# intel/hexl-fpga

Measured on AMD Instinct MI355X. Metric: keyswitches/sec at N=16384, decomp=7, higher is better.
Workload: dtype u64; 1 GPU; keyswitch N=16384 decomp_modulus_size=7 key_modulus_size=8 52-bit primes (GeneratePrimes(K,51,N)), kcc=2, batch 8192 per step split over 1 GPU(s) (8192 on rank 0), resident in HBM; global_batch=8192, batch_per_gpu=8192, parallelism=1 independent shard(s), no collective

## Files before the change

### hexl-fpga_amd/__init__.py

```python
from __future__ import annotations

import ctypes
import os
import subprocess
from pathlib import Path

import numpy as np

_PKG = Path(__file__).resolve().parent
ROOT = _PKG.parent
LIB_PATH = Path(os.environ["HEXL_MI355X_LIB"]) if os.environ.get("HEXL_MI355X_LIB") else _PKG / "lib" / "libhexl_mi355x.so"

_u64 = ctypes.c_uint64
_sz = ctypes.c_size_t
_vp = ctypes.c_void_p
_i = ctypes.c_int

C_ABI = {
    "hexl_device_count": [],
    "hexl_ctx_create": [_i, ctypes.POINTER(_vp)],
    "hexl_ctx_destroy": [_vp],
    "hexl_ctx_set_stream": [_vp, _vp],
    "hexl_ctx_use_own_stream": [_vp],
    "hexl_ctx_sync": [_vp],
    "hexl_ctx_describe": [_vp, ctypes.c_char_p, _sz],
    "hexl_ntt_fwd": [_vp, _vp, _sz, _vp, _vp, _u64, _u64],
    "hexl_ntt_inv": [_vp, _vp, _sz, _vp, _vp, _u64, _u64, _u64, _u64],
    "hexl_dyadic_multiply": [_vp, _vp, _vp, _vp, _sz, _u64, _vp, _u64],
    "hexl_ks_plan_create": [_vp, _u64, _u64, _u64, _u64, _u64, _vp, _vp, _vp, ctypes.POINTER(_vp)],
    "hexl_ks_plan_destroy": [_vp],
    "hexl_ks_set_keys": [_vp, ctypes.POINTER(_vp)],
    "hexl_keyswitch": [_vp, _vp, _vp, _sz],
    "hexl_ks_range_check": [_vp],
    "hexl_ks_plan_tiers": [_vp, ctypes.POINTER(_i)],
    "hexl_multiply_relinearize": [_vp, _vp, _vp, _vp, _sz],
    "hexl_apply_galois": [_vp, _vp, _vp, _sz, _u64, _u64],
    "hexl_rescale": [_vp, _vp, _vp, _sz, _u64, _u64],
    "hexl_rotate": [_vp, _vp, _vp, _sz, _u64],
    "hexl_rotate_hoisted": [ctypes.POINTER(_vp), ctypes.POINTER(_u64), _sz, ctypes.POINTER(_vp), _vp, _sz],
    "hexl_linear_transform": [ctypes.POINTER(_vp), ctypes.POINTER(_u64), ctypes.POINTER(_vp), _sz, _vp, _vp, _vp, _sz],
    "hexl_linear_transform_bsgs": [ctypes.POINTER(_vp), ctypes.POINTER(_u64), _sz, ctypes.POINTER(_vp), ctypes.POINTER(_u64), _sz,
                                   ctypes.POINTER(_vp), ctypes.POINTER(_vp), _vp, _vp, _sz],
    "hexl_lt_bsgs_scratch_bytes": [_vp, _sz, _sz],
    "hexl_rns_ntt_fwd": [_vp, _vp, _vp, _sz, _u64],
    "hexl_rns_ntt_inv": [_vp, _vp, _vp, _sz, _u64],
    "hexl_multiply_plain": [_vp, _vp, _vp, _vp, _sz, _u64, _u64, _sz, _i],
    "hexl_ks_scratch_bytes": [_vp, _sz],
    "hexl_ntt_fwd_host": [_vp, ctypes.POINTER(_vp), _sz, _vp, _vp, _u64, _u64],
    "hexl_ntt_inv_host": [_vp, ctypes.POINTER(_vp), _sz, _vp, _vp, _u64, _u64, _u64, _u64],
    "hexl_dyadic_multiply_host": [_vp, ctypes.POINTER(_vp), ctypes.POINTER(_vp), ctypes.POINTER(_vp), _sz, _u64,
                                  ctypes.POINTER(_vp), _u64],
    "hexl_keyswitch_host": [_vp, ctypes.POINTER(_vp), ctypes.POINTER(_vp), _sz],
    "hexl_ks_time_stages": [_vp, _vp, _vp, _sz, _i, ctypes.POINTER(ctypes.c_float)],
}


class HexlError(RuntimeError):
    pass


def build(force: bool = False) -> Path:
    if force or not LIB_PATH.exists():
        subprocess.run(["make", "-C", str(_PKG / "csrc"), "-j4"] + (["-B"] if force else []), check=True)
    else:
        subprocess.run(["make", "-C", str(_PKG / "csrc"), "-j4", "-s"], check=True)
    return LIB_PATH

# ... 96 lines not shown
    def __init__(self, ctx: Context, n: int, L: int, K: int, rns: int, kcc: int, moduli, modswitch,
                 twiddles=None):
        self.ctx, self.n, self.L, self.K = ctx, n, L, K
        mod = np.ascontiguousarray(moduli, dtype=np.uint64)
        msf = np.ascontiguousarray(modswitch, dtype=np.uint64)
        tw = None if twiddles is None else np.ascontiguousarray(twiddles, dtype=np.uint64)
        h = _vp()
        _check(lib().hexl_ks_plan_create(ctx.h, n, L, K, rns, kcc, mod.ctypes.data, msf.ctypes.data,
                                         None if tw is None else tw.ctypes.data, ctypes.byref(h)),
               "hexl_ks_plan_create")
        self.h = h

    def set_keys(self, keys):
        self._keys = [np.ascontiguousarray(k, dtype=np.uint64) for k in keys]
        arr = (_vp * len(self._keys))(*[k.ctypes.data for k in self._keys])
        _check(lib().hexl_ks_set_keys(self.h, arr), "hexl_ks_set_keys")

    def keyswitch(self, result, t_target, batch: int):
        _check(lib().hexl_keyswitch(self.h, _ptr(result), _ptr(t_target), batch), "hexl_keyswitch")

    def range_check(self) -> bool:
        rc = lib().hexl_ks_range_check(self.h)
        if rc not in (0, 1):
            _check(rc, "hexl_ks_range_check")
        return rc == 0

    def tiers(self):
        out = (_i * self.K)()
        rc = lib().hexl_ks_plan_tiers(self.h, out)
        if rc not in (0, 1):
            _check(rc, "hexl_ks_plan_tiers")
        return list(out), rc == 1

    def multiply_relinearize(self, out, a, b, batch: int):
        _check(lib().hexl_multiply_relinearize(self.h, _ptr(out), _ptr(a), _ptr(b), batch), "hexl_multiply_relinearize")

    def rescale(self, out, inp, batch: int, n_limbs: int, n_components: int):
        _check(lib().hexl_rescale(self.h, _ptr(out), _ptr(inp), batch, n_limbs, n_components), "hexl_rescale")

    def rotate(self, out, ct, batch: int, g: int):
        _check(lib().hexl_rotate(self.h, _ptr(out), _ptr(ct), batch, g), "hexl_rotate")

    def rns_ntt_fwd(self, out, inp, count: int, n_limbs: int):
        _check(lib().hexl_rns_ntt_fwd(self.h, _ptr(out), _ptr(inp), count, n_limbs), "hexl_rns_ntt_fwd")

    def rns_ntt_inv(self, out, inp, count: int, n_limbs: int):
        _check(lib().hexl_rns_ntt_inv(self.h, _ptr(out), _ptr(inp), count, n_limbs), "hexl_rns_ntt_inv")

    def multiply_plain(self, out, ct, pt, batch: int, n_components: int, n_limbs: int, pt_batch: int, accumulate: bool = False):
        _check(lib().hexl_multiply_plain(self.h, _ptr(out), _ptr(ct), _ptr(pt), batch, n_components, n_limbs, pt_batch,
                                         1 if accumulate else 0), "hexl_multiply_plain")

    def keyswitch_host(self, results, t_targets):
        n = len(results)
        r = (_vp * n)(*[_ptr(a) for a in results])
        t = (_vp * n)(*[_ptr(a) for a in t_targets])
        rc = lib().hexl_keyswitch_host(self.h, r, t, n)
        if rc != 1:
            _check(rc, "hexl_keyswitch_host")
        return rc == 0

    def time_stages(self, result, t_target, batch: int, iters: int):
        out = (ctypes.c_float * 4)()
        _check(lib().hexl_ks_time_stages(self.h, _ptr(result), _ptr(t_target), batch, iters, out),
               "hexl_ks_time_stages")
        return list(out)
# ... 57 lines not shown
```

### hexl-fpga_amd/csrc/capi.hip

```cpp
#include <string.h>

#include <atomic>

#include "hexl_internal.hpp"
#include "number_theory.hpp"

int hx_grow_device(void** p, size_t* cap, size_t need, size_t unit, hexl_ctx* ctx) {
    if (*cap >= need) return 0;
    if (*p) {
        HX_CHECK(ctx ? hipStreamSynchronize(ctx->stream) : hipDeviceSynchronize());
        HX_CHECK(hipFree(*p));
        *p = nullptr; *cap = 0;
    }
    HX_CHECK(hipMalloc(p, need * unit));
    *cap = need;
    return 0;
}
int hx_reserve_pinned(hexl_ctx* ctx, void** p, size_t* cur, size_t need, bool coherent) {
    if (*cur >= need) return 0;
    if (*p) { HX_CHECK(hipStreamSynchronize(ctx->stream)); HX_CHECK(hipHostFree(*p)); *p = nullptr; *cur = 0; }
    HX_CHECK(hipHostMalloc(p, need, coherent ? hipHostMallocCoherent : hipHostMallocDefault));
    *cur = need;
    return 0;
}
// ... 164 lines not shown
            hxnt::forward_roots(n, logn, q, w, roots);
            hxnt::inverse_roots_from0(n, q, roots, inv0.data());
        }
        iroots[0] = 1;
        for (u64 r = 1; r < n; ++r) iroots[r] = inv0[r - 1];
        for (u64 r = 0; r < n; ++r) {
            precon[r] = hx_shoup(roots[r], q);
            iprecon[r] = hx_shoup(iroots[r], q);
        }
        KsModulus& m = mods[i];
        m.q = q;
        m.qbarr = (u64)(((u128)1 << 64) / q);
        m.inv_n = hxnt::invmod(n, q);
        m.inv_n_p = hx_shoup(m.inv_n, q);
        m.inv_n_w = hxnt::mulmod(m.inv_n, iroots[n - 1] % q, q);
        m.inv_n_w_p = hx_shoup(m.inv_n_w, q);
        u64 msf = h_modswitch[i];
        if (msf >= 4 * q) msf -= 4 * q;
        if (msf >= 2 * q) msf -= 2 * q;
        if (msf >= q) msf -= q;
        m.msf = msf;
        m.msf_p = hx_shoup(msf, q);
        m.half = q_sp >> 1;
        m.fix = q - (m.half % q);
        u32 fl = 63;
        while (!(q >> fl)) --fl;
        m.len = fl - 1;
        m.barr_lo = (u64)(((u128)1 << (m.len + 64)) / q);
    }
    bool f64_ok = hx_knob("HEXL_KS_INT", 0) != 1;
    for (u64 i = 0; i < K; ++i) f64_ok = f64_ok && h_moduli[i] < (1ULL << 52);
    if (logn == 15 && !f64_ok) return HEXL_E_BADARG;
    p->use_f64 = f64_ok;
    p->f64_lazy = 0;
    p->f64_loge = ks_loge(logn, true);
    p->int_loge = ks_loge(logn, false);
    if (logn == 14) {
        const long e = hx_knob("HEXL_KSI_LOGE", 0);
        if (e == 4 || e == 5) p->int_loge = (u32)e;
    }
    if (f64_ok && hx_knob("HEXL_KS_NOLAZY", 0) != 1) {
        double qmax = 0;
        for (u64 i = 0; i < K; ++i) qmax = (double)h_moduli[i] > qmax ? (double)h_moduli[i] : qmax;
        p->f64_lazy = hxf::lazy_period_for(qmax);
        double qmin = qmax;
        for (u64 i = 0; i < K; ++i) qmin = (double)h_moduli[i] < qmin ? (double)h_moduli[i] : qmin;
        p->x_skip = p->f64_lazy && qmax <= hxf::LAZY_SKIP_MAX_RATIO * qmin && hx_knob("HEXL_KSX_SKIP", 1) != 0;
        const long e = hx_knob("HEXL_KS_PERIOD", 12);
        const int cap = (e == 3 || e == 6) ? (int)e : 12;
        if (p->f64_lazy > cap) p->f64_lazy = cap;
        const bool per_limb = hx_knob_ks_per_limb() != 0;
        for (u64 i = 0; i < K; ++i) {
            int t = per_limb ? hxf::lazy_period_for((double)h_moduli[i]) : p->f64_lazy;
            if (t > cap) t = cap;
            p->tier[i] = (unsigned char)t;
            if ((i < L || i == K - 1) && t != p->f64_lazy) p->mixed = true;
        }
    }
    if (f64_ok) {
        std::vector<KsModF64> fm(K);
        std::vector<double> ft(size_t(K) * 4 * n);
        for (u64 i = 0; i < K; ++i) {
            const u64 q = h_moduli[i];
            const double pd = (double)q;
            auto centre = [&](u64 v) { return hx_centre(v % q, q); };
            for (int blk = 0; blk < 4; blk += 2)
// ... 171 lines not shown
```

### hexl-fpga_amd/csrc/hexl_internal.hpp

```cpp
#pragma once
#include <hip/hip_runtime.h>
#include <limits.h>
#include <stdint.h>
#include <stdio.h>
#include <stdlib.h>

#include <mutex>
#include <type_traits>
#include <vector>

#include "../../include/hexl_mi355x.h"
#include "f64_arith.hpp"

typedef uint64_t u64;
typedef uint32_t u32;
typedef unsigned __int128 u128;

#define HX_CHECK(expr)                                                                       \
    do {                                                                                     \
        hipError_t _e = (expr);                                                              \
        if (_e != hipSuccess) {                                                              \
            fprintf(stderr, "[hexl_mi355x] %s failed: %s (%s:%d)\n", #expr,                  \
                    hipGetErrorString(_e), __FILE__, __LINE__);                              \
            return (int)_e;                                                                  \
// ... 78 lines not shown
    double half;
};

constexpr int HX_KS_MAX_LANES = 4;
int hx_ks_lanes();

struct hexl_ks_plan {
    hexl_ctx* ctx = nullptr;
    u32 n = 0, logn = 0, L = 0, K = 0, rns = 0;
    std::vector<u64> moduli;
    KsModulus* d_mods = nullptr;
    u64* d_tables = nullptr;
    u64* d_keys = nullptr;
    u32 int_loge = 5;
    bool have_keys = false;
    bool use_f64 = false;
    int f64_lazy = 0;
    unsigned char tier[16] = {};
    bool mixed = false;
    u32 f64_loge = 4;
    KsModF64* d_mods_f64 = nullptr;
    double* d_tables_f64 = nullptr;
    double* d_keys_f64 = nullptr;
    double* d_keys_x = nullptr;
    u32 x_loge = 5;
    u64* d_scratch = nullptr;
    size_t cap = 0;
    hipStream_t aux[HX_KS_MAX_LANES] = {};
    hipEvent_t ev_start = nullptr, ev_done[HX_KS_MAX_LANES] = {};
    u32* d_flag = nullptr;
    u32* h_flag = nullptr;
    double* d_keys_nat = nullptr;
    bool x_skip = false;
    bool overwrite_result = false;
    u32* host_done = nullptr;
    u32* host_flag = nullptr;
    u32 host_epoch = 0;
    hipStream_t cur = nullptr;
    u64* cur_scratch = nullptr;
    KsRescaleF64* d_rescale = nullptr;
    u32 rescale_levels = 0;
    double* d_rs_s = nullptr;
    size_t rs_cap = 0;
    u64* d_rot_t = nullptr;
    size_t rot_cap = 0;
    double* d_bsgs_b = nullptr;
    size_t bsgs_b_cap = 0;
    u64* d_bsgs_t = nullptr;
    size_t bsgs_t_cap = 0;
};

int hx_launch_ntt_fwd(hexl_ctx*, u64* d_x, size_t batch, const u64* roots, const u64* precon, u64 q, u64 n);
int hx_launch_ntt_inv(hexl_ctx*, u64* d_x, size_t batch, const u64* iroots, const u64* iprecon, u64 q,
                      u64 inv_n, u64 inv_n_p, u64 inv_n_w, u64 inv_n_w_p, u64 n);
int hx_launch_dyadic(hexl_ctx*, u64* d_out, const u64* d_a, const u64* d_b, size_t batch, u64 n,
                     const u64* d_moduli, u64 n_moduli);
int hx_launch_keyswitch(hexl_ks_plan*, u64* d_result, const u64* d_t_target, size_t batch, int stage_mask,
                        hipEvent_t* ev );
int hx_launch_keyswitch_f64(hexl_ks_plan*, u64* d_result, const u64* d_t_target, size_t nb, int stage_mask,
                            hipEvent_t* ev);
int hx_launch_keyswitch_x(hexl_ks_plan*, u64* d_result, const u64* d_t_target, size_t nb, int stage_mask,
                          hipEvent_t* ev);
bool hx_ks_x_applies(const hexl_ks_plan*, size_t nb);
size_t hx_ks_chunk(const hexl_ks_plan*);
bool hx_ks_chunk_forced();
bool hx_ks_can_overwrite(const hexl_ks_plan*, size_t nb);
// ... 63 lines not shown
```

### hexl-fpga_amd/csrc/keyswitch.hip

```cpp
#include <stdlib.h>

#ifndef HX_IFWD_PRIO
#define HX_IFWD_PRIO 1222
#endif
#include "hexl_internal.hpp"
#include "ntt_core.hpp"

using namespace hx;

__device__ __forceinline__ u64 barrett64(u64 v, u64 q, u64 qbarr) {
    return csub(v - mulhi(v, qbarr) * q, q);
}
__device__ __forceinline__ u64 mulmod128(u64 x, u64 y, u64 q, u32 len, u64 barr_lo) {
    const u64 lo = x * y, hi = mulhi(x, y);
    const u64 c1 = (lo >> len) | (hi << (64 - len));
    return csub(lo - mulhi(c1, barr_lo) * q, q);
}

__device__ __forceinline__ u32 xcd_item(u32 bid, u32 total) {
    const u32 q = total >> 3, r = total & 7, xcd = bid & 7, j = bid >> 3;
    return xcd * q + (xcd < r ? xcd : r) + j;
}

struct KsArgs {
// ... 332 lines not shown
static size_t scratch_words(const hexl_ks_plan* p) {
    return p->use_f64 ? hx_ks_f64_scratch_words(p->L) : size_t(3) * p->L + 2;
}
int hx_ks_lanes() {
    static const int v = [] { const long l = hx_knob("HEXL_KS_LANES", 2); return l < 2 ? 2 : l > HX_KS_MAX_LANES ? HX_KS_MAX_LANES : (int)l; }();
    return v;
}
static size_t lane_bytes(const hexl_ks_plan* p) { return size_t(hx_ks_lanes()) * scratch_words(p) * p->n * sizeof(u64); }
size_t hexl_ks_scratch_bytes(const hexl_ks_plan* p, size_t batch) { return hx_ks_chunk_of(p, batch) * lane_bytes(p); }
static int reserve_scratch(hexl_ks_plan* p, size_t chunk) {
    return hx_grow_device((void**)&p->d_scratch, &p->cap, chunk, lane_bytes(p), nullptr);
}

__global__ void k_ks_validate(const u64* __restrict__ t, const u64* __restrict__ res, const KsModulus* __restrict__ mods,
                              u32 L, u32 n, size_t batch, u32* __restrict__ bad) {
    const size_t per_t = size_t(L) * n, per_r = 2 * per_t, total = batch * (per_t + (res ? per_r : 0));
    bool out = false;
    for (size_t g = size_t(blockIdx.x) * blockDim.x + threadIdx.x; g < total; g += size_t(gridDim.x) * blockDim.x) {
        u64 word; u32 limb;
        if (g < batch * per_t) { word = t[g]; limb = u32((g % per_t) / n); }
        else { const size_t h = g - batch * per_t; word = res[h]; limb = u32(((h % per_r) / n) % L); }
        out |= word >= mods[limb].q;
    }
    if (out) atomicOr(bad, 1u);
}

static int validate_inputs(hexl_ks_plan* p, const u64* d_result, const u64* d_t_target, size_t batch) {
    HX_CHECK(hipMemsetAsync(p->d_flag + 1, 0, sizeof(u32), p->ctx->stream));
    hipLaunchKernelGGL(k_ks_validate, dim3(2048), dim3(256), 0, p->ctx->stream, d_t_target, p->overwrite_result ? nullptr : d_result,
                       p->d_mods, p->L, p->n, batch, p->d_flag + 1);
    HX_CHECK(hipMemcpyAsync(p->h_flag + 1, p->d_flag + 1, sizeof(u32), hipMemcpyDeviceToHost, p->ctx->stream));
    HX_CHECK(hipStreamSynchronize(p->ctx->stream));
    return p->h_flag[1] ? HEXL_E_RANGE : 0;
}

bool hx_ks_can_overwrite(const hexl_ks_plan* p, size_t nb) {
    if (!p->use_f64 || p->logn > 14) return false;
    const size_t chunk = hx_ks_chunk_of(p, nb);
    return !hx_ks_x_applies(p, chunk) && !hx_ks_x_applies(p, nb % chunk ? nb % chunk : chunk);
}

int hx_launch_keyswitch(hexl_ks_plan* p, u64* d_result, const u64* d_t_target, size_t batch, int stage_mask,
                        hipEvent_t* ev) {
    if (!batch) return 0;
    if (!p->have_keys) return HEXL_E_NOKEYS;
    static const bool validate = hx_knob("HEXL_KS_VALIDATE", 0) == 1;
    if (validate)
        if (int rc = validate_inputs(p, d_result, d_t_target, batch)) return rc;
    size_t chunk = hx_ks_chunk_of(p, batch);
    const long lane_env = hx_knob("HEXL_KS_ONE_LANE", HX_KNOB_UNSET);
    const bool one_lane = lane_env != HX_KNOB_UNSET ? lane_env == 1 : (p->use_f64 && !hx_ks_x_applies(p, chunk));
    const bool two_lanes = !ev && batch >= 64 && !one_lane && !(p->use_f64 && batch <= chunk);
    if (two_lanes && batch <= chunk) chunk = (batch + 1) / 2;
    if (int rc = reserve_scratch(p, chunk)) return rc;
    if (!p->aux[0]) {
        for (int l = 0; l < hx_ks_lanes(); ++l) {
            HX_CHECK(hipStreamCreateWithFlags(&p->aux[l], hipStreamNonBlocking));
            HX_CHECK(hipEventCreateWithFlags(&p->ev_done[l], hipEventDisableTiming));
        }
        HX_CHECK(hipEventCreateWithFlags(&p->ev_start, hipEventDisableTiming));
    }
    hipStream_t user = p->ctx->stream;
    const int lanes = two_lanes ? hx_ks_lanes() : 1;
    if (lanes >= 2) {
        HX_CHECK(hipEventRecord(p->ev_start, user));
        for (int l = 0; l < lanes; ++l) HX_CHECK(hipStreamWaitEvent(p->aux[l], p->ev_start, 0));
// ... 71 lines not shown
```

### hexl-fpga_amd/csrc/keyswitch_x.hip

```cpp
#include <stdlib.h>

#ifndef HX_FWD_PRIO
#define HX_FWD_PRIO 1222
#endif
#include "hexl_internal.hpp"
#include "ntt_core_f64.hpp"

using namespace hx;

#ifndef KX_PRE
#define KX_PRE 11
#endif
#ifndef KX_IPRE
#define KX_IPRE 1
#endif

#define KX_WAVES(LOGE) ((LOGE) == 4 ? 4 : 2)

#ifdef HEXL_PROFILING_AIDS
#define KX_ALIASED(bit, x) ((a.alias & (bit)) ? 0u : (x))
#else
#define KX_ALIASED(bit, x) (x)
#endif

// ... 16 lines not shown
    const u64 *mul_a, *mul_b;
    unsigned long long* stamps;
};

#ifdef KX_TIMELINE
constexpr int KX_NST = 64;
#define KX_STAMP(i)                                                                                            \
    do {                                                                                                       \
        _Pragma("unroll") for (int r_ = 0; r_ < G::E; ++r_) asm volatile("" : "+v"(v[r_]));                    \
        if (a.stamps && (threadIdx.x & 63) == 0)                                                               \
            a.stamps[(size_t(kx_slot) * (G::T / 64) + (threadIdx.x >> 6)) * KX_NST + (i)] = __builtin_readcyclecounter(); \
        _Pragma("unroll") for (int r_ = 0; r_ < G::E; ++r_) asm volatile("" : "+v"(v[r_]));                    \
    } while (0)
#else
#define KX_STAMP(i) do { } while (0)
#endif

struct XcdWalk { u32 pos, end, step; };
__device__ __forceinline__ XcdWalk xcd_walk(u32 total) {
    const u32 g = gridDim.x >> 3, q = total >> 3, r = total & 7, x = blockIdx.x & 7, j = blockIdx.x >> 3;
    const u32 start = x * q + (x < r ? x : r);
    return XcdWalk{start + j, start + q + (x < r ? 1u : 0u), g};
}

__device__ __forceinline__ u32 sel_limb(const KsArgsX& a, u32 j) { return u32(a.selmap >> (4 * j)) & 15u; }

__device__ __forceinline__ KsModF64 load_mod_const(const KsModF64* p) {
    static_assert(sizeof(KsModF64) == 10 * sizeof(double), "KsModF64 is ten doubles");
    const ctw_t q = (ctw_t)(const double*)p;
    KsModF64 f;
    f.m.p = q[0]; f.m.pinv = q[1];
    f.sc.n = q[2]; f.sc.n_p = q[3]; f.sc.nw = q[4]; f.sc.nw_p = q[5];
    f.msf = q[6]; f.msf_p = q[7]; f.fix = q[8]; f.half = q[9];
    return f;
}

template <class G>
__device__ __forceinline__ const double* key_row(const KsArgsX& a, u32 d, u32 slot) {
    return a.keys + size_t(d * (a.L + 1) + slot) * a.key_stride;
}

__device__ __forceinline__ u32 xcd_item_x(u32 bid, u32 total) {
    const u32 q = total >> 3, r = total & 7, xcd = bid & 7, j = bid >> 3;
    return xcd * q + (xcd < r ? xcd : r) + j;
}

template <class G>
__device__ __forceinline__ void load_natural_to_B(double (&v)[G::E], const u64* __restrict__ src, double* lds, int tid,
                                                  const Mod m, hxf::RangeMask& bad) {
    if constexpr (G::KL <= 2) {
        const u32 tB = u32(G::idxB(0, tid));
#pragma unroll
        for (int r = 0; r < G::E; ++r) v[r] = hxf::reduce(hxf::to_f64_checked((src + G::idxB(r, 0))[tB], m, bad), m);
    } else {
#pragma unroll
        for (int r = 0; r < G::E; ++r) v[r] = hxf::reduce(hxf::to_f64_checked((src + G::idxA(r, 0))[u32(tid)], m, bad), m);
        redeal_x<G, false, true>(v, lds, tid, [](int r, int t) { return G::idxA(r, t); },
                                 [](int r, int t) { return G::idxB(r, t); });
    }
}

#ifndef KX_PF_DEPTH
#define KX_PF_DEPTH 3
#endif
constexpr int KX_PF = KX_PF_DEPTH;
#ifndef KX_SEMI_UNI
// ... 277 lines not shown
                (res + G::idxB(r0 + r, 0))[tB] = hxf::from_f64(hxf::lift(rr, m));
            }
            __builtin_amdgcn_sched_barrier(0);
        }
        return;
    }
    double* const atA = lds + G::pad(G::idxA(0, tid));
    double* const atB = lds + G::pad(G::idxB(0, tid));
    __syncthreads();
    auto old_at_A = [&](int r) {
        auto ld = [&](const u64* p) { return hxf::reduce(hxf::to_f64((p + G::idxA(r, 0))[u32(tid)]), m); };
        if constexpr (FUSED_K == 0) return hxf::mul_mod(ld(a0), ld(b0), m);
        else if constexpr (FUSED_K == 1) return hxf::reduce(hxf::mul_mod(ld(a0), ld(b1), m) + hxf::mul_mod(ld(a1), ld(b0), m), m);
        else return hxf::reduce(hxf::to_f64_checked((res + G::idxA(r, 0))[u32(tid)], m, bad), m);
    };
#pragma unroll
    for (int r0 = 0; r0 < G::E; r0 += (FUSED_K == 1 ? 4 : 8)) {
#pragma unroll
        for (int r = r0; r < r0 + (FUSED_K == 1 ? 4 : 8); ++r) atA[G::pad(G::idxA(r, 0))] = old_at_A(r);
        __builtin_amdgcn_sched_barrier(0);
    }
    __syncthreads();
#pragma unroll
    for (int r = 0; r < G::E; ++r) {
        const double o = atB[G::pad(G::idxB(r, 0))];
        atB[G::pad(G::idxB(r, 0))] = hxf::lift(hxf::reduce(o + v[r], m), m);
    }
    __syncthreads();
#pragma unroll
    for (int r = 0; r < G::E; ++r) (res + G::idxA(r, 0))[u32(tid)] = hxf::from_f64(atA[G::pad(G::idxA(r, 0))]);
}

template <int LOGN, int LOGE, int LAZY, bool FUSED = false, bool SKIP = false>
__global__ __launch_bounds__(1 << (LOGN - LOGE), KX_WAVES(LOGE)) void k_ksx_main(KsArgsX a) {
    using G = Geom<LOGN, LOGE>;
    static_assert(!SKIP || LAZY != 0, "SKIP is a lazy-kernel variant");
    using W = WgNttF64<LOGN, LOGE, LAZY, KsxDownOpt<LAZY>>;
    using WU = WgNttF64<LOGN, LOGE, LAZY, KsxUpOpt<LAZY, SKIP>>;
    constexpr bool LAZYFOLD = LAZY != 0;
    extern __shared__ __attribute__((aligned(16))) double ldsx[];
    const u32 L = a.L;
    {
    const u32 item = __builtin_amdgcn_readfirstlane(xcd_item_x(blockIdx.x, gridDim.x));
#ifdef KX_TIMELINE
    const u32 kx_slot = item;
#endif
    const u32 b = item / a.nsel, i = sel_limb(a, item - b * a.nsel);
    const KsModF64 md = load_mod_const(a.mods + i);
    const Mod m = md.m;
    const u32 bc = KX_ALIASED(2, b), bt = KX_ALIASED(4, b), br = KX_ALIASED(8, b);
    auto round_src = [&](u32 it) { return it < L ? a.c + (size_t(bc) * L + it) * G::N : a.s + (size_t(bc) * 2 + (it - L)) * G::N; };
    const u32 first = i == 0 ? 1u : 0u;
    double acc0[G::E], acc1[G::E];
    double v[G::E];
    {
        int tid = threadIdx.x;
        asm volatile("" : "+v"(tid));
        const double* k0 = key_row<G>(a, i, i);
        KX_STAMP(60);
        if constexpr (!FUSED && G::KL <= 2) {
            KX_STAMP(61);
            mac_keys_first<G, LAZYFOLD>(acc0, acc1, v, a.t_target + (size_t(bt) * L + i) * G::N, k0, round_src(first), tid, m);
        } else {
#pragma unroll
            for (int r = 0; r < G::E; ++r) { acc0[r] = 0.0; acc1[r] = 0.0; }
            if constexpr (FUSED) {
                const size_t at = ((size_t(b) * 2 + 1) * L + i) * G::N;
                load_product_to_B<G>(v, a.mul_a + at, a.mul_b + at, ldsx, tid, m);
            } else {
                hxf::RangeMask ignore = 0;
                load_natural_to_B<G>(v, a.t_target + (size_t(bt) * L + i) * G::N, ldsx, tid, m, ignore);
            }
            KX_STAMP(61);
            mac_keys<G>(acc0, acc1, v, k0, round_src(first), tid, m);
        }
    }
#pragma unroll 1
    for (u32 it = first; it < L;) {
        int tid = threadIdx.x;
        asm volatile("" : "+v"(tid));
        u32 toff = KX_ALIASED(16, i) * 4 * G::N;
        asm volatile("" : "+s"(toff));
        const double* tb = a.tables + toff;
        KX_STAMP(4 * it + 0);
        if constexpr (!SKIP) {
#pragma unroll
            for (int r = 0; r < G::E; ++r) v[r] = hxf::reduce(v[r], m);
        }
        KX_STAMP(4 * it + 1);
        u32 nit = it + 1;
        if (nit == i) ++nit;
        const double* k0 = key_row<G>(a, it, i);
        WU::template forward<false, false>(v, ldsx, tid, tb, tb + G::N, m);
        KX_STAMP(4 * it + 2);
        mac_keys<G, true>(acc0, acc1, v, k0, round_src(nit), tid, m);
        it = nit;
    }
    if constexpr (LAZY == 0) {
#pragma unroll
        for (int r = 0; r < G::E; ++r) { acc0[r] = hxf::reduce(acc0[r], m); acc1[r] = hxf::reduce(acc1[r], m); }
    }
    hxf::RangeMask bad = 0;
    {
        int tid = threadIdx.x;
        asm volatile("" : "+v"(tid));
        u32 toff = KX_ALIASED(16, i) * 4 * G::N;
        asm volatile("" : "+s"(toff));
        const double* tb = a.tables + toff;
        KX_STAMP(4 * L + 0);
        const size_t o0 = ((size_t(br) * 2 + 0) * L + i) * G::N, o1 = ((size_t(br) * 2 + 1) * L + i) * G::N;
        if constexpr (FUSED) ksx_down_round<G, W, 0, SKIP>(v, acc0, a.result + o0, ldsx, tid, tb, md, bad, a.mul_a + o0, a.mul_a + o1, a.mul_b + o0, a.mul_b + o1);
        else ksx_down_round<G, W, -1, SKIP>(v, acc0, a.result + o0, ldsx, tid, tb, md, bad);
        const double* nxt = a.s + (size_t(bc) * 2 + 1) * G::N;
#pragma unroll
        for (int r = 0; r < G::E; ++r) v[r] = (nxt + G::idxA(r, 0))[u32(tid)];
        KX_STAMP(4 * L + 4);
    }
    {
        int tid = threadIdx.x;
        asm volatile("" : "+v"(tid));
        u32 toff = KX_ALIASED(16, i) * 4 * G::N;
        asm volatile("" : "+s"(toff));
        const double* tb = a.tables + toff;
        const size_t o0 = ((size_t(br) * 2 + 0) * L + i) * G::N, o1 = ((size_t(br) * 2 + 1) * L + i) * G::N;
        if constexpr (FUSED) ksx_down_round<G, W, 1, SKIP>(v, acc1, a.result + o1, ldsx, tid, tb, md, bad, a.mul_a + o0, a.mul_a + o1, a.mul_b + o0, a.mul_b + o1);
        else ksx_down_round<G, W, -1, SKIP>(v, acc1, a.result + o1, ldsx, tid, tb, md, bad);
        KX_STAMP(4 * L + 8);
        hxf::report_range(bad, a.range_flag);
    }
    }
}

constexpr int KSH_HB = 8;
template <class G, int LAZY, bool SKIP, int SHIFT, unsigned XS = 0u>
__device__ __forceinline__ void ksh_combine(double (&v)[G::E], const double* __restrict__ hi_row, int tid, const double* w, const Mod m, u32 h) {
    const double W1 = ((ctw_t)w)[1];
    constexpr bool red = XS ? false : (LAZY == 0 || hxf::lazy_fwd_reduce_after(1, 15, LAZY ? LAZY : 3, SHIFT));
    constexpr int HB = KSH_HB;
#pragma unroll
    for (int r0 = 0; r0 < G::E; r0 += HB) {
        double hi[HB];
#pragma unroll
        for (int r = 0; r < HB; ++r) hi[r] = (hi_row + G::idxA(r0 + r, 0))[u32(tid)];
#pragma unroll
        for (int r = 0; r < HB; ++r) {
            double lo = v[r0 + r], y = hi[r];
            if constexpr (!SKIP) { lo = hxf::reduce(lo, m); y = hxf::reduce(y, m); }
            const double t = hxf::mul_mod(y, W1, m);
            const double o = h ? lo - t : lo + t;
            v[r0 + r] = red ? hxf::reduce(o, m) : o;
        }
        __builtin_amdgcn_sched_barrier(0);
    }
}

template <int LAZY, bool FUSED = false>
__global__ __launch_bounds__(1024, 4) void k_ksh_intt(KsArgsX a) {
    using G = Geom<14, 4>;
    using W = WgNttF64<14, 4, LAZY, InvNoWpOpt<false, 1>>;
    constexpr u32 NF = 2 * G::N;
    extern __shared__ __attribute__((aligned(16))) double ldsx[];
    const XcdWalk wk = xcd_walk(a.nb * a.nsel * 2);
// ... 156 lines not shown
        asm volatile("" : "+v"(tid));
        u32 toff = i * 4 * NF;
        asm volatile("" : "+s"(toff));
        const double* tb = a.tables + toff;
        ksh_combine<G, LAZY, SKIP, 0, W::XS>(v, round_src(L) + G::N, tid, tb, m, h);
        const size_t o0 = ((size_t(b) * 2 + 0) * L + i) * NF + h * G::N, o1 = ((size_t(b) * 2 + 1) * L + i) * NF + h * G::N;
        if constexpr (FUSED) ksx_down_round<G, W, 0, SKIP, true>(v, acc0, a.result + o0, ldsx, tid, tb, md, bad, a.mul_a + o0, a.mul_a + o1, a.mul_b + o0, a.mul_b + o1, h);
        else ksx_down_round<G, W, -1, SKIP, true>(v, acc0, a.result + o0, ldsx, tid, tb, md, bad, nullptr, nullptr, nullptr, nullptr, h);
        const double* nxt = round_src(L + 1);
#pragma unroll
        for (int r = 0; r < G::E; ++r) v[r] = (nxt + G::idxA(r, 0))[u32(tid)];
    }
    {
        int tid = threadIdx.x;
        asm volatile("" : "+v"(tid));
        u32 toff = i * 4 * NF;
        asm volatile("" : "+s"(toff));
        const double* tb = a.tables + toff;
        ksh_combine<G, LAZY, SKIP, 0, W::XS>(v, round_src(L + 1) + G::N, tid, tb, m, h);
        const size_t o0 = ((size_t(b) * 2 + 0) * L + i) * NF + h * G::N, o1 = ((size_t(b) * 2 + 1) * L + i) * NF + h * G::N;
        if constexpr (FUSED) ksx_down_round<G, W, 1, SKIP, true>(v, acc1, a.result + o1, ldsx, tid, tb, md, bad, a.mul_a + o0, a.mul_a + o1, a.mul_b + o0, a.mul_b + o1, h);
        else ksx_down_round<G, W, -1, SKIP, true>(v, acc1, a.result + o1, ldsx, tid, tb, md, bad, nullptr, nullptr, nullptr, nullptr, h);
    }
    hxf::report_range(bad, a.range_flag);
}

template <int LOGN, int LOGE, int LAZY, bool FUSED = false, bool SKIP = false>
static int launch_stage_x(hexl_ks_plan* p, const KsArgsX& a, int stage) {
    using G = Geom<LOGN, LOGE>;
    if (int rc = hx_lds_optin<k_ksx_special<LOGN, LOGE, LAZY, SKIP>, k_ksx_intt<LOGN, LOGE, LAZY, FUSED>, k_ksx_main<LOGN, LOGE, LAZY, FUSED, SKIP>>(
            p->ctx->device, G::LDS_USED))
        return rc;
    hipStream_t st = p->cur;
    static const int persist = (int)hx_knob("HEXL_KSX_PERSIST", 1);
    constexpr u32 wg_per_cu = (KX_WAVES(LOGE) * 4 * 64) / G::T ? (KX_WAVES(LOGE) * 4 * 64) / G::T : 1;
    auto grid_for = [&](u32 items) {
        const u32 per_xcd = (items + 7) / 8, slots = (((u32)p->ctx->num_cu + 7) / 8) * wg_per_cu;
        return dim3(8 * (persist && per_xcd > slots ? slots : per_xcd));
    };
    if (stage == 1)
        hipLaunchKernelGGL((k_ksx_intt<LOGN, LOGE, LAZY, FUSED>), grid_for(a.nb * a.nsel), dim3(G::T), G::LDS_USED, st, a);
    if (stage == 2)
        hipLaunchKernelGGL((k_ksx_special<LOGN, LOGE, LAZY, SKIP>), grid_for(a.nb), dim3(G::T), G::LDS_USED, st, a);
    if (stage == 4)
        hipLaunchKernelGGL((k_ksx_main<LOGN, LOGE, LAZY, FUSED, SKIP>), dim3(a.nb * a.nsel), dim3(G::T), G::LDS_USED, st, a);
    return 0;
}

template <int LOGN, int LOGE, bool FUSED>
static int launch_stage_tier(hexl_ks_plan* p, const KsArgsX& a, int stage, int tier, bool skip) {
    if constexpr (LOGN == 14 && LOGE == 4 && !FUSED) {
        switch (tier * 2 + (skip && tier ? 1 : 0)) {
            case 25: return launch_stage_x<14, 4, 12, false, true>(p, a, stage);
            case 24: return launch_stage_x<14, 4, 12>(p, a, stage);
            case 13: return launch_stage_x<14, 4, 6, false, true>(p, a, stage);
            case 12: return launch_stage_x<14, 4, 6>(p, a, stage);
            case 7:  return launch_stage_x<14, 4, 3, false, true>(p, a, stage);
            case 6:  return launch_stage_x<14, 4, 3>(p, a, stage);
            default: return launch_stage_x<14, 4, 0>(p, a, stage);
        }
    } else {
        if (!tier) return launch_stage_x<LOGN, LOGE, 0, FUSED>(p, a, stage);
        return skip ? launch_stage_x<LOGN, LOGE, 3, FUSED, true>(p, a, stage) : launch_stage_x<LOGN, LOGE, 3, FUSED>(p, a, stage);
    }
}

template <class Key, class Launch>
static int per_group(KsArgsX& a, Key key, Launch launch) {
    bool done[16] = {};
    for (u32 i0 = 0; i0 < a.L; ++i0) {
        if (done[i0]) continue;
        a.nsel = 0; a.selmap = 0;
        for (u32 i = i0; i < a.L; ++i)
            if (!done[i] && key(i) == key(i0)) { done[i] = true; a.selmap |= (unsigned long long)i << (4 * a.nsel++); }
        if (int rc = launch(key(i0))) return rc;
    }
    return 0;
}
// ... 129 lines not shown
```

### include/hexl_mi355x.h

```cpp
#ifndef HEXL_MI355X_H
#define HEXL_MI355X_H

#include <stddef.h>
#include <stdint.h>

#ifdef __cplusplus
extern "C" {
#endif

#define HEXL_E_BADARG   (-1)
#define HEXL_E_NOKEYS   (-2)
#define HEXL_E_NODEVICE (-3)
#define HEXL_E_RANGE    (-4)
#define HEXL_W_RANGE    1

typedef struct hexl_ctx hexl_ctx;
typedef struct hexl_ks_plan hexl_ks_plan;

int hexl_device_count(void);

int hexl_ctx_create(int device, hexl_ctx** out);
int hexl_ctx_destroy(hexl_ctx* ctx);
int hexl_ctx_set_stream(hexl_ctx* ctx, void* hip_stream);
int hexl_ctx_use_own_stream(hexl_ctx* ctx);
// ... 11 lines not shown
                         const uint64_t* d_b, size_t batch, uint64_t n,
                         const uint64_t* d_moduli, uint64_t n_moduli);

int hexl_ks_plan_create(hexl_ctx* ctx, uint64_t n, uint64_t decomp_modulus_size,
                        uint64_t key_modulus_size, uint64_t rns_modulus_size,
                        uint64_t key_component_count, const uint64_t* h_moduli,
                        const uint64_t* h_modswitch, const uint64_t* h_twiddles,
                        hexl_ks_plan** out);
int hexl_ks_plan_destroy(hexl_ks_plan* plan);
int hexl_ks_set_keys(hexl_ks_plan* plan, const uint64_t* const* h_keys);
int hexl_keyswitch(hexl_ks_plan* plan, uint64_t* d_result, const uint64_t* d_t_target,
                   size_t batch);
int hexl_ks_range_check(hexl_ks_plan* plan);
int hexl_multiply_relinearize(hexl_ks_plan* plan, uint64_t* d_out, const uint64_t* d_a,
                              const uint64_t* d_b, size_t batch);
int hexl_apply_galois(hexl_ctx* ctx, uint64_t* d_out, const uint64_t* d_in, size_t count, uint64_t n, uint64_t galois_elt);
int hexl_rescale(hexl_ks_plan* plan, uint64_t* d_out, const uint64_t* d_in, size_t batch, uint64_t n_limbs,
                 uint64_t n_components);
int hexl_rotate(hexl_ks_plan* plan, uint64_t* d_out, const uint64_t* d_ct, size_t batch, uint64_t galois_elt);
int hexl_rotate_hoisted(hexl_ks_plan* const* plans, const uint64_t* galois_elts, size_t n_rot, uint64_t* const* d_outs,
                        const uint64_t* d_ct, size_t batch);
int hexl_linear_transform(hexl_ks_plan* const* plans, const uint64_t* galois_elts, const uint64_t* const* d_pts, size_t n_rot,
                          const uint64_t* d_pt_identity, uint64_t* d_out, const uint64_t* d_ct, size_t batch);
int hexl_linear_transform_bsgs(hexl_ks_plan* const* baby_plans, const uint64_t* baby_elts, size_t n_baby,
                               hexl_ks_plan* const* giant_plans, const uint64_t* giant_elts, size_t n_giant,
                               const uint64_t* const* d_pts, const uint64_t* const* d_pt_identity, uint64_t* d_out,
                               const uint64_t* d_ct, size_t batch);
size_t hexl_lt_bsgs_scratch_bytes(const hexl_ks_plan* plan, size_t n_baby, size_t batch);
int hexl_rns_ntt_fwd(hexl_ks_plan* plan, uint64_t* d_out, const uint64_t* d_in, size_t count, uint64_t n_limbs);
int hexl_rns_ntt_inv(hexl_ks_plan* plan, uint64_t* d_out, const uint64_t* d_in, size_t count, uint64_t n_limbs);
int hexl_multiply_plain(hexl_ks_plan* plan, uint64_t* d_out, const uint64_t* d_ct, const uint64_t* d_pt, size_t batch,
                        uint64_t n_components, uint64_t n_limbs, size_t pt_batch, int accumulate);
int hexl_ks_plan_tiers(const hexl_ks_plan* plan, int* tiers );
size_t hexl_ks_scratch_bytes(const hexl_ks_plan* plan, size_t batch);

int hexl_ntt_fwd_host(hexl_ctx* ctx, uint64_t* const* h_x, size_t batch, const uint64_t* h_roots,
                      const uint64_t* h_precon, uint64_t q, uint64_t n);
int hexl_ntt_inv_host(hexl_ctx* ctx, uint64_t* const* h_x, size_t batch, const uint64_t* h_inv_roots,
                      const uint64_t* h_inv_precon, uint64_t q, uint64_t inv_n,
                      uint64_t inv_n_w, uint64_t n);
int hexl_dyadic_multiply_host(hexl_ctx* ctx, uint64_t* const* h_out, const uint64_t* const* h_a,
                              const uint64_t* const* h_b, size_t batch, uint64_t n,
                              const uint64_t* const* h_moduli, uint64_t n_moduli);
int hexl_keyswitch_host(hexl_ks_plan* plan, uint64_t* const* h_results,
                        const uint64_t* const* h_t_targets, size_t batch);

int hexl_ks_time_stages(hexl_ks_plan* plan, uint64_t* d_result, const uint64_t* d_t_target,
                        size_t batch, int iters, float* ms_out );

#ifdef __cplusplus
}
#endif
#endif
```

Before: 220,900 keyswitches/s.

## Make keyswitch main kernel persistent and reload kernel args per phase

Converts k_ksx_main from one workgroup per (batch, limb) item into a persistent kernel that walks items in an XCD-aware stride loop, launched with a grid sized to CU slots. Kernel arguments are re-read from the kernarg segment in each phase rather than held live across the kernel, which lowers SGPR/VGPR pressure. It also moves the persist knob into the plan and adds a query API that reports which pipeline path applies. The persistent loop avoids per-workgroup launch and scheduling overhead, but it can cause load imbalance, and the repeated scalar loads add a small cost.

```diff
diff --git a/hexl-fpga_amd/__init__.py b/hexl-fpga_amd/__init__.py
--- a/hexl-fpga_amd/__init__.py
+++ b/hexl-fpga_amd/__init__.py
@@ -33,6 +33,7 @@
     "hexl_keyswitch": [_vp, _vp, _vp, _sz],
     "hexl_ks_range_check": [_vp],
     "hexl_ks_plan_tiers": [_vp, ctypes.POINTER(_i)],
+    "hexl_ks_plan_pipeline": [_vp, _sz],
     "hexl_multiply_relinearize": [_vp, _vp, _vp, _vp, _sz],
     "hexl_apply_galois": [_vp, _vp, _vp, _sz, _u64, _u64],
     "hexl_rescale": [_vp, _vp, _vp, _sz, _u64, _u64],
@@ -195,6 +196,12 @@
             _check(rc, "hexl_ks_plan_tiers")
         return list(out), rc == 1
 
+    def pipeline(self, batch: int) -> int:
+        rc = lib().hexl_ks_plan_pipeline(self.h, batch)
+        if rc < 0:
+            _check(rc, "hexl_ks_plan_pipeline")
+        return rc
+
     def multiply_relinearize(self, out, a, b, batch: int):
         _check(lib().hexl_multiply_relinearize(self.h, _ptr(out), _ptr(a), _ptr(b), batch), "hexl_multiply_relinearize")
 
diff --git a/hexl-fpga_amd/csrc/capi.hip b/hexl-fpga_amd/csrc/capi.hip
--- a/hexl-fpga_amd/csrc/capi.hip
+++ b/hexl-fpga_amd/csrc/capi.hip
@@ -220,6 +220,7 @@
     for (u64 i = 0; i < K; ++i) f64_ok = f64_ok && h_moduli[i] < (1ULL << 52);
     if (logn == 15 && !f64_ok) return HEXL_E_BADARG;
     p->use_f64 = f64_ok;
+    p->x_persist = hx_knob("HEXL_KSX_PERSIST", 1) != 0;
     p->f64_lazy = 0;
     p->f64_loge = ks_loge(logn, true);
     p->int_loge = ks_loge(logn, false);
diff --git a/hexl-fpga_amd/csrc/hexl_internal.hpp b/hexl-fpga_amd/csrc/hexl_internal.hpp
--- a/hexl-fpga_amd/csrc/hexl_internal.hpp
+++ b/hexl-fpga_amd/csrc/hexl_internal.hpp
@@ -134,6 +134,7 @@
     u32* h_flag = nullptr;
     double* d_keys_nat = nullptr;
     bool x_skip = false;
+    bool x_persist = true;
     bool overwrite_result = false;
     u32* host_done = nullptr;
     u32* host_flag = nullptr;
diff --git a/hexl-fpga_amd/csrc/keyswitch.hip b/hexl-fpga_amd/csrc/keyswitch.hip
--- a/hexl-fpga_amd/csrc/keyswitch.hip
+++ b/hexl-fpga_amd/csrc/keyswitch.hip
@@ -388,6 +388,14 @@
     HX_CHECK(hipMemcpyAsync(p->h_flag + 1, p->d_flag + 1, sizeof(u32), hipMemcpyDeviceToHost, p->ctx->stream));
     HX_CHECK(hipStreamSynchronize(p->ctx->stream));
     return p->h_flag[1] ? HEXL_E_RANGE : 0;
+}
+
+extern "C" int hexl_ks_plan_pipeline(const hexl_ks_plan* p, size_t batch) {
+    if (!p || !batch) return HEXL_E_BADARG;
+    if (!p->use_f64) return 0;
+    const size_t chunk = hx_ks_chunk_of(p, batch);
+    const bool full = hx_ks_x_applies(p, chunk), tail = hx_ks_x_applies(p, batch % chunk ? batch % chunk : chunk);
+    return full && tail ? 2 : (full || tail ? 3 : 1);
 }
 
 bool hx_ks_can_overwrite(const hexl_ks_plan* p, size_t nb) {
diff --git a/hexl-fpga_amd/csrc/keyswitch_x.hip b/hexl-fpga_amd/csrc/keyswitch_x.hip
--- a/hexl-fpga_amd/csrc/keyswitch_x.hip
+++ b/hexl-fpga_amd/csrc/keyswitch_x.hip
@@ -72,6 +72,20 @@
     f.m.p = q[0]; f.m.pinv = q[1];
     f.sc.n = q[2]; f.sc.n_p = q[3]; f.sc.nw = q[4]; f.sc.nw_p = q[5];
     f.msf = q[6]; f.msf_p = q[7]; f.fix = q[8]; f.half = q[9];
+    return f;
+}
+
+__device__ __forceinline__ KsArgsX reload_args() {
+    static_assert(sizeof(KsArgsX) % 8 == 0, "KsArgsX is read as 64-bit words");
+    constexpr int NW = sizeof(KsArgsX) / 8;
+    unsigned long long at = (unsigned long long)__builtin_amdgcn_kernarg_segment_ptr();
+    asm volatile("" : "+s"(at));
+    const auto* q = (const __attribute__((address_space(4))) unsigned long long*)at;
+    unsigned long long w[NW];
+#pragma unroll
+    for (int k = 0; k < NW; ++k) w[k] = q[k];
+    KsArgsX f;
+    __builtin_memcpy(&f, w, sizeof(f));
     return f;
 }
 
@@ -415,35 +429,47 @@
 }
 
 template <int LOGN, int LOGE, int LAZY, bool FUSED = false, bool SKIP = false>
-__global__ __launch_bounds__(1 << (LOGN - LOGE), KX_WAVES(LOGE)) void k_ksx_main(KsArgsX a) {
+__global__ __launch_bounds__(1 << (LOGN - LOGE), KX_WAVES(LOGE)) void k_ksx_main(KsArgsX launch) {
     using G = Geom<LOGN, LOGE>;
     static_assert(!SKIP || LAZY != 0, "SKIP is a lazy-kernel variant");
     using W = WgNttF64<LOGN, LOGE, LAZY, KsxDownOpt<LAZY>>;
     using WU = WgNttF64<LOGN, LOGE, LAZY, KsxUpOpt<LAZY, SKIP>>;
     constexpr bool LAZYFOLD = LAZY != 0;
     extern __shared__ __attribute__((aligned(16))) double ldsx[];
-    const u32 L = a.L;
-    {
-    const u32 item = __builtin_amdgcn_readfirstlane(xcd_item_x(blockIdx.x, gridDim.x));
+    const XcdWalk wk = xcd_walk(launch.nb * launch.nsel);
+#pragma unroll 1
+    for (u32 item_ = wk.pos; item_ < wk.end; item_ += wk.step) {
+    const u32 item = __builtin_amdgcn_readfirstlane(item_);
 #ifdef KX_TIMELINE
     const u32 kx_slot = item;
 #endif
-    const u32 b = item / a.nsel, i = sel_limb(a, item - b * a.nsel);
-    const KsModF64 md = load_mod_const(a.mods + i);
-    const Mod m = md.m;
+#define KX_PHASE_ARGS                                      \
+    const KsArgsX a = reload_args();                       \
+    const u32 L = a.L;                                     \
+    const KsModF64 md = load_mod_const(a.mods + i);        \
+    const Mod m = md.m
+    u32 b, i;
+    {
+        const KsArgsX a = reload_args();
+        b = item / a.nsel;
+        i = sel_limb(a, item - b * a.nsel);
+    }
     const u32 bc = KX_ALIASED(2, b), bt = KX_ALIASED(4, b), br = KX_ALIASED(8, b);
-    auto round_src = [&](u32 it) { return it < L ? a.c + (size_t(bc) * L + it) * G::N : a.s + (size_t(bc) * 2 + (it - L)) * G::N; };
+    auto round_src = [bc](const KsArgsX& a, u32 it) {
+        return it < a.L ? a.c + (size_t(bc) * a.L + it) * G::N : a.s + (size_t(bc) * 2 + (it - a.L)) * G::N;
+    };
     const u32 first = i == 0 ? 1u : 0u;
     double acc0[G::E], acc1[G::E];
     double v[G::E];
     {
+        KX_PHASE_ARGS;
         int tid = threadIdx.x;
         asm volatile("" : "+v"(tid));
         const double* k0 = key_row<G>(a, i, i);
         KX_STAMP(60);
         if constexpr (!FUSED && G::KL <= 2) {
             KX_STAMP(61);
-            mac_keys_first<G, LAZYFOLD>(acc0, acc1, v, a.t_target + (size_t(bt) * L + i) * G::N, k0, round_src(first), tid, m);
+            mac_keys_first<G, LAZYFOLD>(acc0, acc1, v, a.t_target + (size_t(bt) * L + i) * G::N, k0, round_src(a, first), tid, m);
         } else {
 #pragma unroll
             for (int r = 0; r < G::E; ++r) { acc0[r] = 0.0; acc1[r] = 0.0; }
@@ -455,11 +481,14 @@
                 load_natural_to_B<G>(v, a.t_target + (size_t(bt) * L + i) * G::N, ldsx, tid, m, ignore);
             }
             KX_STAMP(61);
-            mac_keys<G>(acc0, acc1, v, k0, round_src(first), tid, m);
-        }
-    }
+            mac_keys<G>(acc0, acc1, v, k0, round_src(a, first), tid, m);
+        }
+    }
+    u32 it = first;
 #pragma unroll 1
-    for (u32 it = first; it < L;) {
+    for (;;) {
+        KX_PHASE_ARGS;
+        if (it >= L) break;
         int tid = threadIdx.x;
         asm volatile("" : "+v"(tid));
         u32 toff = KX_ALIASED(16, i) * 4 * G::N;
@@ -476,15 +505,17 @@
         const double* k0 = key_row<G>(a, it, i);
         WU::template forward<false, false>(v, ldsx, tid, tb, tb + G::N, m);
         KX_STAMP(4 * it + 2);
-        mac_keys<G, true>(acc0, acc1, v, k0, round_src(nit), tid, m);
+        mac_keys<G, true>(acc0, acc1, v, k0, round_src(a, nit), tid, m);
         it = nit;
     }
     if constexpr (LAZY == 0) {
+        KX_PHASE_ARGS;
 #pragma unroll
         for (int r = 0; r < G::E; ++r) { acc0[r] = hxf::reduce(acc0[r], m); acc1[r] = hxf::reduce(acc1[r], m); }
     }
     hxf::RangeMask bad = 0;
     {
+        KX_PHASE_ARGS;
         int tid = threadIdx.x;
         asm volatile("" : "+v"(tid));
         u32 toff = KX_ALIASED(16, i) * 4 * G::N;
@@ -500,6 +531,7 @@
         KX_STAMP(4 * L + 4);
     }
     {
+        KX_PHASE_ARGS;
         int tid = threadIdx.x;
         asm volatile("" : "+v"(tid));
         u32 toff = KX_ALIASED(16, i) * 4 * G::N;
@@ -511,6 +543,7 @@
         KX_STAMP(4 * L + 8);
         hxf::report_range(bad, a.range_flag);
     }
+#undef KX_PHASE_ARGS
     }
 }
 
@@ -733,7 +766,7 @@
             p->ctx->device, G::LDS_USED))
         return rc;
     hipStream_t st = p->cur;
-    static const int persist = (int)hx_knob("HEXL_KSX_PERSIST", 1);
+    const bool persist = p->x_persist;
     constexpr u32 wg_per_cu = (KX_WAVES(LOGE) * 4 * 64) / G::T ? (KX_WAVES(LOGE) * 4 * 64) / G::T : 1;
     auto grid_for = [&](u32 items) {
         const u32 per_xcd = (items + 7) / 8, slots = (((u32)p->ctx->num_cu + 7) / 8) * wg_per_cu;
@@ -744,7 +777,7 @@
     if (stage == 2)
         hipLaunchKernelGGL((k_ksx_special<LOGN, LOGE, LAZY, SKIP>), grid_for(a.nb), dim3(G::T), G::LDS_USED, st, a);
     if (stage == 4)
-        hipLaunchKernelGGL((k_ksx_main<LOGN, LOGE, LAZY, FUSED, SKIP>), dim3(a.nb * a.nsel), dim3(G::T), G::LDS_USED, st, a);
+        hipLaunchKernelGGL((k_ksx_main<LOGN, LOGE, LAZY, FUSED, SKIP>), grid_for(a.nb * a.nsel), dim3(G::T), G::LDS_USED, st, a);
     return 0;
 }
 
diff --git a/include/hexl_mi355x.h b/include/hexl_mi355x.h
--- a/include/hexl_mi355x.h
+++ b/include/hexl_mi355x.h
@@ -67,6 +67,7 @@
 int hexl_multiply_plain(hexl_ks_plan* plan, uint64_t* d_out, const uint64_t* d_ct, const uint64_t* d_pt, size_t batch,
                         uint64_t n_components, uint64_t n_limbs, size_t pt_batch, int accumulate);
 int hexl_ks_plan_tiers(const hexl_ks_plan* plan, int* tiers );
+int hexl_ks_plan_pipeline(const hexl_ks_plan* plan, size_t batch);
 size_t hexl_ks_scratch_bytes(const hexl_ks_plan* plan, size_t batch);
 
 int hexl_ntt_fwd_host(hexl_ctx* ctx, uint64_t* const* h_x, size_t batch, const uint64_t* h_roots,
```

Result: slower. 213,200 keyswitches/s (-3.5%).
